# hrdkjain/GenIcoNet

Measured on AMD Instinct MI355X. Metric: meshes/sec training throughput, ico2ico I5 batch=36, higher is better.
Workload: dtype f32; 1 GPU; ico2ico AE training, I5, batch 36 per GPU (BASELINE configs[1]); per_gpu_batch=36, global_batch=36, subdivisions=5, parallelism=dp1

## Files before the change

geniconet_amd/_lib.py:

```python
import ctypes
import os

import numpy as np

_HERE = os.path.dirname(os.path.abspath(__file__))
LIB_PATH = os.environ.get('ICN_LIB_PATH') or os.path.join(_HERE, 'libicn.so')

OP_CONV_FWD, OP_CONV_BWD_DATA, OP_CONV_BWD_WEIGHT = 0, 1, 2
CORNER_MODES = {'zeros': 0, 'average': 1}
ABI_VERSION = 9
LAP_MODES = {'mean-v': 0, 'v-mean': 1, 'sum-kv': 2, 'kv-sum': 3}

_c_float_p = ctypes.c_void_p
_i32p = ctypes.POINTER(ctypes.c_int32)
_f32p = ctypes.POINTER(ctypes.c_float)
_intp = ctypes.POINTER(ctypes.c_int)

SIGNATURES = {
    'icn_abi_version': (ctypes.c_int, []),
    'icn_last_error': (ctypes.c_char_p, []),
    'icn_prepare_conv': (ctypes.c_int, [ctypes.c_int] * 3),
    'icn_prepare_upsample': (ctypes.c_int, [ctypes.c_int] * 2),
    'icn_conv_workspace_bytes': (ctypes.c_size_t, [ctypes.c_int] * 6),
    'icn_conv_fwd': (ctypes.c_int, [_c_float_p] * 4 + [ctypes.c_int] * 6 + [ctypes.c_void_p, ctypes.c_size_t, ctypes.c_void_p]),
# ... 23 lines not shown
    'icn_head_bwd': (ctypes.c_int, [_c_float_p] * 8 + [ctypes.c_int] * 3 + [ctypes.c_void_p]),
    'icn_p2p_loss_workspace_floats': (ctypes.c_size_t, [ctypes.c_int] * 2),
    'icn_p2p_loss_fwd': (ctypes.c_int, [_c_float_p] * 2 + [ctypes.c_int] * 2 + [ctypes.c_float] * 3 + [ctypes.c_int] + [_c_float_p] * 2 + [ctypes.c_void_p]),
    'icn_p2p_loss_bwd_workspace_floats': (ctypes.c_size_t, [ctypes.c_int] * 2),
    'icn_p2p_loss_bwd': (ctypes.c_int, [_c_float_p] * 3 + [ctypes.c_int] * 2 + [ctypes.c_float] * 3 + [ctypes.c_int] + [_c_float_p] * 2 + [ctypes.c_void_p]),
    'icn_mesh_reg_workspace_floats': (ctypes.c_size_t, [ctypes.c_int] * 2),
    'icn_mesh_reg_fwd': (ctypes.c_int, [_c_float_p] + [ctypes.c_int] * 2 + [ctypes.c_float] * 4 + [_c_float_p] * 2 + [ctypes.c_void_p]),
    'icn_mesh_reg_bwd_workspace_floats': (ctypes.c_size_t, [ctypes.c_int] * 2),
    'icn_mesh_reg_bwd': (ctypes.c_int, [_c_float_p] * 2 + [ctypes.c_int] * 2 + [ctypes.c_float] * 4 + [_c_float_p] * 2 + [ctypes.c_void_p]),
    'icn_kld_workspace_floats': (ctypes.c_size_t, [ctypes.c_size_t]),
    'icn_kld_fwd': (ctypes.c_int, [_c_float_p] * 2 + [ctypes.c_size_t] + [_c_float_p] * 2 + [ctypes.c_void_p]),
    'icn_kld_bwd': (ctypes.c_int, [_c_float_p] * 3 + [ctypes.c_size_t] + [_c_float_p] * 2 + [ctypes.c_void_p]),
    'icn_reparam_fwd': (ctypes.c_int, [_c_float_p] * 3 + [ctypes.c_size_t] + [_c_float_p] + [ctypes.c_void_p]),
    'icn_reparam_bwd': (ctypes.c_int, [_c_float_p] * 3 + [ctypes.c_size_t] + [_c_float_p] * 2 + [ctypes.c_void_p]),
    'icn_adam_step': (ctypes.c_int, [ctypes.c_int] + [ctypes.c_void_p] * 7 + [ctypes.c_double] * 4 + [ctypes.c_void_p]),
    'icn_adam_step_dev': (ctypes.c_int, [ctypes.c_int] + [ctypes.c_void_p] * 6 + [ctypes.c_double] * 4 + [ctypes.c_void_p]),
    'icn_table_stream_k': (ctypes.c_long, [ctypes.c_int] * 4 + [_i32p, ctypes.c_size_t]),
    'icn_table_tile_lists': (ctypes.c_long, [ctypes.c_int] * 7 + [_i32p, ctypes.c_size_t]),
    'icn_set_debug_flags': (ctypes.c_int, [ctypes.c_int]),
    'icn_device_status': (ctypes.c_int, [ctypes.c_int]),
    'icn_get_arith': (ctypes.c_int, []),
    'icn_set_arith': (ctypes.c_int, [ctypes.c_int]),
    'icn_build_flags': (ctypes.c_uint, []),
    'icn_host_selfcheck': (ctypes.c_long, [ctypes.c_int] * 2),
    'icn_debug_trace': (ctypes.c_int, [ctypes.c_void_p, ctypes.c_size_t]),
    'icn_point_to_mesh': (ctypes.c_int, [_c_float_p] * 3 + [ctypes.c_int] * 4 + [_c_float_p] * 3 + [ctypes.c_void_p]),
    'icn_point_to_mesh_bwd_workspace_bytes': (ctypes.c_size_t, [ctypes.c_int] * 4),
    'icn_point_to_mesh_grid_workspace_bytes': (ctypes.c_size_t, [ctypes.c_int] * 4),
    'icn_point_to_mesh_grid': (ctypes.c_int, [_c_float_p] * 3 + [ctypes.c_int] * 4 + [_c_float_p] * 3 + [ctypes.c_void_p, ctypes.c_size_t, ctypes.c_void_p]),
    'icn_point_to_mesh_bwd': (ctypes.c_int, [_c_float_p] * 6 + [ctypes.c_int] * 4 + [_c_float_p] * 2 + [ctypes.c_void_p, ctypes.c_size_t, ctypes.c_void_p]),
    'icn_table_conv_fwd': (ctypes.c_long, [ctypes.c_int] * 3 + [_i32p, ctypes.c_size_t]),
    'icn_table_wgrad7': (ctypes.c_long, [ctypes.c_int] * 3 + [_i32p, ctypes.c_size_t, ctypes.POINTER(ctypes.c_uint16), ctypes.c_size_t, _intp]),
    'icn_table_conv_bwd': (ctypes.c_long, [ctypes.c_int] * 3 + [_i32p, ctypes.c_size_t, _intp]),
    'icn_table_upsample': (ctypes.c_long, [ctypes.c_int] * 3 + [_i32p, _f32p, ctypes.c_size_t, _intp]),
    'icn_table_upsample_pairs': (ctypes.c_long, [ctypes.c_int, _i32p, ctypes.c_size_t]),
    'icn_table_faces': (ctypes.c_long, [ctypes.c_int, _i32p, ctypes.c_size_t]),
    'icn_table_vertex_stencils': (ctypes.c_long, [ctypes.c_int, _i32p, ctypes.c_size_t]),
    'icn_table_upconv_bwd': (ctypes.c_long, [ctypes.c_int] * 2 + [_i32p, _f32p, ctypes.c_size_t, _intp]),
    'icn_table_upconv': (ctypes.c_long, [ctypes.c_int, ctypes.c_int, _i32p, ctypes.c_size_t, _f32p, ctypes.c_size_t, _intp]),
}



class ProfileEntry(ctypes.Structure):
    _fields_ = [('kernel', ctypes.c_char_p), ('launches', ctypes.c_long), ('total_ms', ctypes.c_double),
                ('total_flops', ctypes.c_double)]


SIGNATURES['icn_profile_start'] = (ctypes.c_int, [ctypes.c_int])
SIGNATURES['icn_profile_stop'] = (ctypes.c_int, [ctypes.POINTER(ProfileEntry), ctypes.c_int])
SIGNATURES['icn_profile_select'] = (ctypes.c_int, [ctypes.c_char_p])

_lib = None


def lib():
    global _lib
    if _lib is None:
        if not os.path.exists(LIB_PATH):
            raise RuntimeError(
                'geniconet_amd: %s is missing -- the HIP extension is the product and has no fallback. '
                'Build it with `python -c "import __graft_entry__ as g; g.build()"` '
                '(or `make -C geniconet_amd/csrc`).' % LIB_PATH)
        handle = ctypes.CDLL(LIB_PATH)
        for name, (res, args) in SIGNATURES.items():
            fn = getattr(handle, name)
# ... 88 lines not shown
    n = L.icn_table_conv_fwd(r_in, stride, m, None, 0)
    if n < 0:
        check(-1, 'icn_table_conv_fwd')
    out = np.empty(n, dtype=np.int32)
    L.icn_table_conv_fwd(r_in, stride, m, out.ctypes.data_as(_i32p), n)
    return out.reshape(7, -1)


def table_wgrad7(r_in, stride, corner_mode):
    L, m = lib(), corner_code(corner_mode)
    meta = (ctypes.c_int * 2)()
    n = L.icn_table_wgrad7(r_in, stride, m, None, 0, None, 0, meta)
    if n < 0:
        check(-1, 'icn_table_wgrad7')
    if n == 0:
        return None
    U, npatch = meta[0], meta[1]
    rows, pos = np.empty(n, dtype=np.int32), np.empty(npatch * 16 * 8, dtype=np.uint16)
    L.icn_table_wgrad7(r_in, stride, m, rows.ctypes.data_as(_i32p), n, pos.ctypes.data_as(ctypes.POINTER(ctypes.c_uint16)), pos.size, meta)
    return rows.reshape(npatch, U), pos.reshape(npatch, 16, 8)


def table_conv_bwd(r_in, stride, corner_mode):
    L, m = lib(), corner_code(corner_mode)
    w = ctypes.c_int(0)
    n = L.icn_table_conv_bwd(r_in, stride, m, None, 0, ctypes.byref(w))
    if n < 0:
        check(-1, 'icn_table_conv_bwd')
    out = np.empty(n, dtype=np.int32)
    L.icn_table_conv_bwd(r_in, stride, m, out.ctypes.data_as(_i32p), n, ctypes.byref(w))
    return out.reshape(7, w.value, -1)


def table_upsample(r_in, corner_mode, transpose=False):
    L, m = lib(), corner_code(corner_mode)
    w = ctypes.c_int(0)
    n = L.icn_table_upsample(r_in, m, int(transpose), None, None, 0, ctypes.byref(w))
    if n < 0:
        check(-1, 'icn_table_upsample')
    idx, coef = np.empty(n, dtype=np.int32), np.empty(n, dtype=np.float32)
    L.icn_table_upsample(r_in, m, int(transpose), idx.ctypes.data_as(_i32p), coef.ctypes.data_as(_f32p), n, ctypes.byref(w))
    return idx.reshape(-1, w.value), coef.reshape(-1, w.value)


def table_faces(r):
    L = lib()
    n = L.icn_table_faces(r, None, 0)
    if n < 0:
        check(-1, 'icn_table_faces')
    out = np.empty(n, dtype=np.int32)
    L.icn_table_faces(r, out.ctypes.data_as(_i32p), n)
    return out.reshape(-1, 3)


def table_vertex_stencils(r):
    L = lib()
    n = L.icn_table_vertex_stencils(r, None, 0)
    if n < 0:
        check(-1, 'icn_table_vertex_stencils')
    out = np.empty(n, dtype=np.int32)
    L.icn_table_vertex_stencils(r, out.ctypes.data_as(_i32p), n)
    return out.reshape(-1, 6, 3)


def table_upsample_pairs(r_in):
    L = lib()
# ... 70 lines not shown
```

geniconet_amd/csrc/icn_api.cpp:

```cpp
#include <hip/hip_runtime.h>

#include <algorithm>
#include <cmath>
#include <cstdio>
#include <cstdlib>
#include <cstring>
#include <map>
#include <mutex>
#include <stdexcept>
#include <string>
#include <tuple>
#include <vector>

#include "../../include/icn.h"
#include "icn_geometry.h"
#include "icn_launch.h"
#include "icn_streamk.h"

namespace {

thread_local std::string g_err;

int fail(const std::string& msg) {
    g_err = msg;
// ... 17 lines not shown
        g_dry_elems += v.size();
        return d;
    }
    ICN_HIP(hipMalloc(reinterpret_cast<void**>(&d), v.size() * sizeof(T)));
    ICN_HIP(hipMemcpy(d, v.data(), v.size() * sizeof(T), hipMemcpyHostToDevice));
    return d;
}

struct DevDma {
    int32_t* code = nullptr;
    int32_t* slots = nullptr;
    int n_slots = 0, E = 1;
};
DevDma upload_dma(const std::vector<int32_t>& idx, int E, int P) {
    icn::DmaTable h;
    icn::build_dma_table(idx, E, P, h);
    DevDma d;
    d.code = upload(h.code);
    d.slots = upload(h.slots);
    d.n_slots = h.n_slots;
    d.E = E;
    return d;
}
struct ConvTables {
    int Pin = 0, Pout = 0, n_in = 0, n_out = 0, E = 1;
    int32_t* fwd = nullptr;
    int32_t* bwd = nullptr;
    int32_t* bwd1 = nullptr;
    int nv = 0, nvp = 0;
    int32_t* vidx = nullptr;
    int32_t* vorder = nullptr;
    uint32_t* vmask32 = nullptr;
    int32_t* vq = nullptr;
    int32_t* perm = nullptr;
    int32_t* bwd_perm = nullptr;
    uint32_t* mask32 = nullptr;
    std::vector<uint32_t> mask32_h;
    int key = 0;
    DevDma d_fwd, d_bwd, d_bwd1, d_virt, d_bwdp;
    int32_t* w7_rows = nullptr;
    uint16_t* w7_pos = nullptr;
    int w7_U = 0;
};
struct UpTables {
    int Pc = 0, Pf = 0, Wf = 0, Wb = 0;
    int32_t *idx_f = nullptr, *idx_b = nullptr;
    float *coef_f = nullptr, *coef_b = nullptr;
};

struct UpconvDev {
    int Pc = 0, Pf = 0, n_slots = 0, E = 1, nseg = 0;
    int seg_cnt[icn::UPCONV_MAX_SEG] = {}, seg_off[icn::UPCONV_MAX_SEG] = {};
    uint32_t seg_mask[icn::UPCONV_MAX_SEG] = {};
    int32_t *pix = nullptr, *code = nullptr, *slot_idx = nullptr;
    float *alpha = nullptr, *slot_coef = nullptr;
};

struct EllSplitDev {
    int W = 0, n_ovf = 0, W_ovf = 0;
    int32_t *idx = nullptr, *ovf_rows = nullptr, *ovf_idx = nullptr;
    float *coef = nullptr, *ovf_coef = nullptr;
};
EllSplitDev upload_ell_split(const icn::Ell& e, int W_main) {
    EllSplitDev d;
    const int W = e.width;
    d.W = W_main;
// ... 109 lines not shown
    std::vector<int32_t> fwd, bwd, perm;
    std::vector<uint8_t> mask;
    icn::build_conv_fwd(r_in, stride, mode, fwd);
    t.E = icn::build_conv_bwd(r_in, stride, mode, bwd);
    t.fwd = upload(fwd);
    t.bwd = upload(bwd);
    t.d_fwd = upload_dma(fwd, 1, t.Pout);
    t.d_bwd = upload_dma(bwd, t.E, t.Pin);
    {
        icn::DmaTable h;
        icn::build_dma_table(fwd, 1, t.Pout, h);
        icn::Wg7Table w7;
        if (icn::build_wgrad7(h, t.Pout, wgrad7_union_rows(stride), w7)) {
            t.w7_rows = upload(w7.urow);
            t.w7_pos = upload(w7.upos);
            t.w7_U = w7.U;
        }
    }
    std::vector<int32_t> primary;
    icn::VirtualRows vr;
    icn::split_conv_bwd(r_in, stride, bwd, t.E, primary, vr);
    t.bwd1 = upload(primary);
    t.d_bwd1 = upload_dma(primary, 1, t.Pin);
    t.nv = vr.nv;
    if (vr.nv > 0) {
        std::vector<int32_t> order, vidx_o;
        std::vector<uint8_t> vmask;
        icn::build_virtual_order(vr, t.nvp, order, vidx_o, vmask);
        t.vidx = upload(vidx_o);
        t.vorder = upload(order);
        t.vmask32 = upload(std::vector<uint32_t>(vmask.begin(), vmask.end()));
        t.d_virt = upload_dma(vidx_o, 1, t.nvp);
        t.vq = upload(vr.vq);
    }
    if (stride == 2) {
        icn::build_bwd_row_order(r_in, stride, bwd, t.E, perm, mask);
        t.perm = upload(perm);
        t.mask32_h.assign(mask.begin(), mask.end());
        t.mask32 = upload(t.mask32_h);
        t.key = 1 + ((r_in << 8) | (stride << 4) | mode);
        std::vector<int32_t> bwd_p(bwd.size());
        for (int te = 0; te < icn::NTAPS * t.E; ++te)
            for (int k = 0; k < t.Pin; ++k) bwd_p[(size_t)te * t.Pin + k] = bwd[(size_t)te * t.Pin + perm[k]];
        t.bwd_perm = upload(bwd_p);
        t.d_bwdp = upload_dma(bwd_p, t.E, t.Pin);
    }
    return t;
}
const ConvTables& conv_tables(int r_in, int stride, int mode) {
    int dev = 0;
    ICN_HIP(hipGetDevice(&dev));
    std::lock_guard<std::mutex> lk(g_mu);
    auto key = std::make_tuple(dev, r_in, stride, mode);
    auto it = g_conv.find(key);
    if (it != g_conv.end()) return it->second;
    return g_conv.emplace(key, make_conv_tables(r_in, stride, mode)).first->second;
}

std::map<std::pair<int, int>, int32_t*> g_vf;

const int32_t* vertex_faces(int r) {
    int dev = 0;
    ICN_HIP(hipGetDevice(&dev));
    std::lock_guard<std::mutex> lk(g_mu);
    auto key = std::make_pair(dev, r);
    auto it = g_vf.find(key);
// ... 298 lines not shown
    float* sk_part = reinterpret_cast<float*>(reinterpret_cast<char*>(sk_flag) + align256((size_t)icn::CONV_SK_FLAGS * sizeof(int)));
    icn::PrologueArgs p{};
    p.zero = sk_flag; p.n_zero = icn::CONV_SK_FLAGS;
    p.w = w0; p.w2 = w1; p.packed = wf; p.Cout = C0; p.Cout2 = C1; p.Cin = Cin; p.transpose = 0;
    p.bias = b0; p.bias2 = b1; p.bias_cat = bias_cat;
    p.src = x; p.slots = t.d_fwd.slots; p.side = side; p.n_slots = t.d_fwd.n_slots; p.E = 1; p.B = B; p.Ps = t.Pin; p.K = Cin;
    p.ns = t.n_in;
    icn::GatherGemmArgs a{};
    a.src = x; a.bias = w1 ? bias_cat : b0; a.dst = y0; a.dst2 = w1 ? y1 : nullptr; a.N0 = C0;
    a.idx = t.fwd; a.dcode = t.d_fwd.code; a.side = side; a.n_slots = t.d_fwd.n_slots;
    a.M = B * t.Pout; a.Ps = t.Pin; a.Pd = t.Pout; a.K = Cin; a.N = C; a.E = 1; a.ns = t.n_in;
    a.algo_flops = 2.0 * 7 * Cin * C * (double)B * t.Pout;
    a.sk_part = sk_part; a.sk_flag = sk_flag;
    choose_arith(a, p, wf, (size_t)7 * Cin * C, false);
    icn::launch_conv_prologue(p, s);
    icn::launch_gather_gemm_auto(a, s);
}

void conv_bwd_data_impl(const float* dy0, const float* dy1, const float* w0, const float* w1, float* dx, int B, int Cin, int C0,
                        int C1, int r_in, int stride, const ConvTables& t, void* ws, hipStream_t s) {
    const int C = C0 + C1;
    const size_t wbytes = wpack_bytes((size_t)7 * Cin * C);
    const TableCounts tc = table_counts(r_in, stride);
    const size_t side_bytes = align256((size_t)B * tc.slots_bwd * C0 * sizeof(float));
    float* wb = static_cast<float*>(ws);
    float* vout = reinterpret_cast<float*>(at(ws, wbytes));
    float* side = reinterpret_cast<float*>(at(ws, wbytes + align256((size_t)B * tc.nv * Cin * sizeof(float))));
    float* side2 = dy1 ? reinterpret_cast<float*>(reinterpret_cast<char*>(side) + side_bytes) : nullptr;
    int* sk_flag = reinterpret_cast<int*>(reinterpret_cast<char*>(side) + (dy1 ? 2 : 1) * side_bytes);
    float* sk_part = reinterpret_cast<float*>(reinterpret_cast<char*>(sk_flag) + align256((size_t)icn::CONV_SK_FLAGS * sizeof(int)));
    const bool split = stride == 1 && t.nv > 0 && t.nv * 8 < t.Pin;
    const DevDma& dm = split ? t.d_bwd1 : (stride == 2 ? t.d_bwdp : t.d_bwd);
    const DevDma& ds = split ? t.d_virt : dm;
    icn::PrologueArgs p{};
    p.w = w0; p.w2 = w1; p.packed = wb; p.Cout = C0; p.Cout2 = C1; p.Cin = Cin; p.transpose = 1;
    p.src = dy0; p.src2 = dy1; p.slots = ds.slots; p.side = side; p.side2 = side2; p.n_slots = ds.n_slots; p.E = ds.E; p.B = B;
    p.Ps = t.Pout; p.K = C0; p.ns = t.n_out;
    p.zero = sk_flag; p.n_zero = icn::CONV_SK_FLAGS;
    icn::GatherGemmArgs a{};
    a.src = dy0; a.src2 = dy1; a.dst = dx; a.N0 = Cin;
    a.idx = split ? t.bwd1 : (stride == 2 ? t.bwd_perm : t.bwd); a.dcode = dm.code; a.side = side; a.side2 = side2;
    a.n_slots = dm.n_slots; a.perm = t.perm; a.mask32 = t.mask32;
    a.mask32_host = t.mask32_h.empty() ? nullptr : t.mask32_h.data(); a.mask_key = t.key;
    a.M = B * t.Pin; a.Ps = t.Pout; a.Pd = t.Pin; a.K = C; a.N = Cin; a.E = split ? 1 : t.E; a.ns = t.n_out;
    a.algo_flops = 2.0 * 7 * Cin * C * (double)B * t.Pout;
    a.sk_part = sk_part; a.sk_flag = sk_flag;
    choose_arith(a, p, wb, (size_t)7 * Cin * C, split);
    icn::launch_conv_prologue(p, s);
    icn::launch_gather_gemm_auto(a, s);
    if (split) {
        icn::GatherGemmArgs v = a;
        v.wt = wb; v.arith_bn = 0;
        v.sk_part = nullptr; v.sk_flag = nullptr;
        v.dst = vout; v.idx = t.vidx; v.dcode = t.d_virt.code; v.n_slots = t.d_virt.n_slots; v.perm = t.vorder; v.mask32 = t.vmask32;
        v.M = B * t.nvp; v.Pd = t.nvp; v.E = 1;
        v.algo_flops = 0.0;
        icn::launch_gather_gemm_auto(v, s);
        icn::launch_row_scatter_add(vout, dx, t.vq, B, t.nv, t.nvp, t.Pin, Cin, s);
    }
}

void conv_bwd_weight_impl(const float* x, const float* dy0, const float* dy1, float* dw0, float* db0, float* dw1, float* db1, int B,
                          int Cin, int C0, int C1, const ConvTables& t, void* ws, hipStream_t s) {
    const int C = C0 + C1, M = B * t.Pout;
    float* partial = static_cast<float*>(ws);
    float* bpart = (db0 || db1) ? reinterpret_cast<float*>(at(ws, wgrad_partial_bytes(M, Cin, C, C0))) : nullptr;
    float* side = reinterpret_cast<float*>(at(ws, wgrad_partial_bytes(M, Cin, C, C0) + wgrad_bias_partial_bytes(M, Cin, C, C0)));
    const bool mfma = icn::wgrad_supported(Cin, C);
    if (mfma) {
        icn::PrologueArgs p{};
        p.Cin = Cin; p.src = x; p.slots = t.d_fwd.slots; p.side = side; p.n_slots = t.d_fwd.n_slots; p.E = 1; p.B = B; p.Ps = t.Pin;
        p.K = Cin; p.ns = t.n_in;
        icn::launch_conv_prologue(p, s);
    }
    icn::WgradArgs a{};
    a.x = x; a.dy = dy0; a.dy2 = dy1; a.Cout0 = C0; a.idx = t.fwd; a.dcode = mfma ? t.d_fwd.code : nullptr; a.side = side;
    a.n_slots = t.d_fwd.n_slots; a.partial = partial; a.bias_partial = bpart; a.dw = dw0; a.dbias = db0; a.dw2 = dw1; a.dbias2 = db1;
    a.M = M; a.Ps = t.Pin; a.Pd = t.Pout; a.Cin = Cin; a.Cout = C; a.ns = t.n_in;
    a.algo_flops = 2.0 * 7 * Cin * C * (double)M;
    a.w7_rows = t.w7_rows; a.w7_pos = t.w7_pos; a.w7_U = t.w7_U;
    icn::launch_wgrad(a, s);
}

}

namespace icn {
const char* const PROF_NAMES[PROF_KINDS] = {"k_conv_dma<128, 128, false>", "k_conv_dma<128, 64, false>", "k_conv_dma<64, 128, false>",
                                            "k_conv_dma<64, 64, false>",
                                            "k_gather_gemm<128, 128>", "k_gather_gemm<128, 64>", "k_gather_gemm<64, 128>",
                                            "k_gather_gemm<64, 64>", "k_wgrad_dma<128, 128>", "k_wgrad_dma<128, 64>",
                                            "k_wgrad_dma<64, 128>", "k_wgrad_dma<64, 64>", "k_wgrad<128, 128>", "k_wgrad<128, 64>",
                                            "k_wgrad<64, 128>", "k_wgrad<64, 64>", "k_conv_dma<128, 128, true>",
                                            "k_conv_dma<128, 64, true>", "k_conv_dma<64, 128, true>", "k_conv_dma<64, 64, true>",
                                            "k_conv_dma_sk<64, 128, false>", "k_conv_dma_sk<64, 64, false>", "k_conv_dma_sk<64, 128, true>",
                                            "k_conv_dma_sk<64, 64, true>", "k_wgrad7",
                                            "k_conv_dma8<64, 128, false>", "k_conv_dma8<64, 128, true>", "k_conv_dma_sk8<64, 128, false>",
                                            "k_conv_dma_sk8<64, 128, true>", "k_conv_dense_sk<64, 128>", "k_conv_dense_sk<64, 64>", "k_conv_single_sk<64, 128>",
                                            "k_conv_single_sk<64, 64>", "k_wgrad_dense<128, 128>", "k_wgrad_dense<128, 64>",
                                            "k_wgrad_dense<64, 128>", "k_wgrad_dense<64, 64>",
                                            "k_conv_b3_sk<128, 128, 8>", "k_conv_b3_sk<128, 64, 4>", "k_conv_b3_dense_sk<128, 128, 8>",
                                            "k_conv_b3_dense_sk<128, 64, 4>", "k_wgrad7<.., 1>", "k_wgrad_dma<.., 1>", "k_wgrad_dense<.., 1>", "k_conv_b3<128, BN, NW>",
                                            "k_conv_b3_single_sk<128, 128, 8>", "k_conv_b3_single_sk<128, 64, 4>",
                                            "k_point_to_mesh", "k_point_to_mesh_bwd_point", "k_point_to_mesh_bwd_vertex",
                                            "k_p2m_grid_bounds", "k_p2m_grid_count", "k_p2m_grid_scan", "k_p2m_grid_fill",
                                            "k_p2m_grid_query"};
void prof_mark_begin(int kind, double flops, hipStream_t s) {
    if (!g_prof_on) return;
    g_prof_mu.lock();
    if (!g_prof_on || g_prof_used >= g_prof.size() || (g_prof_only >= 0 && kind != g_prof_only)) { g_prof_mu.unlock(); return; }
    ProfRec& r = g_prof[g_prof_used];
    r.kind = kind;
    r.flops = flops;
    (void)hipEventRecord(r.e0, s);
    g_prof_open = true;
}
void prof_mark_end(hipStream_t s) {
    if (!g_prof_open) return;
    (void)hipEventRecord(g_prof[g_prof_used].e1, s);
    ++g_prof_used;
    g_prof_open = false;
    g_prof_mu.unlock();
}
}

extern "C" {

int icn_profile_start(int max_launches) {
    try {
        if (max_launches < 1) throw std::invalid_argument("icn_profile_start: max_launches must be positive");
        std::lock_guard<std::mutex> lk(g_prof_mu);
        while ((int)g_prof.size() < max_launches) {
            ProfRec r{};
            ICN_HIP(hipEventCreate(&r.e0));
            ICN_HIP(hipEventCreate(&r.e1));
            g_prof.push_back(r);
        }
        g_prof_used = 0;
        g_prof_on = true;
// ... 893 lines not shown

long icn_table_conv_fwd(int r_in, int stride, int corner_mode, int32_t* out, size_t cap) {
    try {
        std::vector<int32_t> v;
        icn::build_conv_fwd(r_in, stride, corner_mode, v);
        if (out) std::memcpy(out, v.data(), std::min(cap, v.size()) * sizeof(int32_t));
        return (long)v.size();
    } catch (const std::exception& e) {
        return fail(e.what());
    }
}

long icn_table_wgrad7(int r_in, int stride, int corner_mode, int32_t* rows, size_t cap_rows, uint16_t* pos, size_t cap_pos, int* meta) {
    try {
        std::vector<int32_t> fwd;
        icn::build_conv_fwd(r_in, stride, corner_mode, fwd);
        const int P = (int)(fwd.size() / icn::NTAPS);
        icn::DmaTable h;
        icn::build_dma_table(fwd, 1, P, h);
        icn::Wg7Table w7;
        if (!icn::build_wgrad7(h, P, wgrad7_union_rows(stride), w7)) {
            if (meta) meta[0] = meta[1] = 0;
            return 0;
        }
        if (meta) { meta[0] = w7.U; meta[1] = w7.npatch; }
        if (rows) std::memcpy(rows, w7.urow.data(), std::min(cap_rows, w7.urow.size()) * sizeof(int32_t));
        if (pos) std::memcpy(pos, w7.upos.data(), std::min(cap_pos, w7.upos.size()) * sizeof(uint16_t));
        return (long)w7.urow.size();
    } catch (const std::exception& e) {
        return fail(e.what());
    }
}

long icn_table_conv_bwd(int r_in, int stride, int corner_mode, int32_t* out, size_t cap, int* width) {
    try {
        std::vector<int32_t> v;
        const int E = icn::build_conv_bwd(r_in, stride, corner_mode, v);
        if (width) *width = E;
        if (out) std::memcpy(out, v.data(), std::min(cap, v.size()) * sizeof(int32_t));
        return (long)v.size();
    } catch (const std::exception& e) {
        return fail(e.what());
    }
}

long icn_table_upsample(int r_in, int corner_mode, int transpose, int32_t* idx, float* coef, size_t cap, int* width) {
    try {
        icn::Ell f, b;
        icn::build_upsample(r_in, corner_mode, f, b);
        const icn::Ell& e = transpose ? b : f;
        if (width) *width = e.width;
        if (idx) std::memcpy(idx, e.idx.data(), std::min(cap, e.idx.size()) * sizeof(int32_t));
        if (coef) std::memcpy(coef, e.coef.data(), std::min(cap, e.coef.size()) * sizeof(float));
        return (long)e.idx.size();
    } catch (const std::exception& e) {
        return fail(e.what());
    }
}

long icn_table_upsample_pairs(int r_in, int32_t* out, size_t cap) {
    try {
        std::vector<int32_t> v;
        icn::build_upsample_pairs(r_in, v);
        if (out) std::memcpy(out, v.data(), std::min(cap, v.size()) * sizeof(int32_t));
        return (long)v.size();
    } catch (const std::exception& e) {
// ... 68 lines not shown
```

geniconet_amd/csrc/icn_geometry.cpp:

```cpp
#include "icn_geometry.h"

#include <algorithm>
#include <cstdlib>
#include <array>
#include <cmath>
#include <map>
#include <stdexcept>

namespace icn {

const int TAP_DA[NTAPS] = {0, 1, 0, -1, -1, 0, 1};
const int TAP_DB[NTAPS] = {0, 0, 1, 1, 0, -1, -1};

namespace {

struct Pt {
    int c, a, b;
};

inline Pt prev1(int, Pt p) { return {(p.c + 4) % 5, p.a + p.b, -p.a}; }
inline Pt prev2(int n, Pt p) { return {(p.c + 4) % 5, p.a + n, p.b - n}; }
inline Pt prev3(int n, Pt p) { return {(p.c + 4) % 5, 3 * n - p.b, p.a + p.b - n}; }
inline Pt next1(int, Pt p) { return {(p.c + 1) % 5, -p.b, p.a + p.b}; }
inline Pt next2(int n, Pt p) { return {(p.c + 1) % 5, p.a - n, p.b + n}; }
// ... 120 lines not shown
        }
        for (size_t l = 0; l < levels; ++l) {
            std::array<int32_t, NTAPS> row;
            for (int t = 0; t < NTAPS; ++t) row[t] = l < leftover[t].size() ? leftover[t][l] : IDX_ZERO;
            rows.push_back(row);
            vr.vq.push_back(q);
        }
    }
    vr.nv = (int)rows.size();
    vr.vidx.assign((size_t)NTAPS * std::max(vr.nv, 1), IDX_ZERO);
    for (int v = 0; v < vr.nv; ++v)
        for (int t = 0; t < NTAPS; ++t) vr.vidx[(size_t)t * vr.nv + v] = rows[v][t];
}

void build_virtual_order(const VirtualRows& vr, int& nvp, std::vector<int32_t>& order, std::vector<int32_t>& vidx_o,
                         std::vector<uint8_t>& mask32) {
    const int nv = vr.nv;
    nvp = (nv + 31) / 32 * 32;
    std::vector<unsigned> taps(nv, 0);
    for (int v = 0; v < nv; ++v)
        for (int t = 0; t < NTAPS; ++t)
            if (vr.vidx[(size_t)t * nv + v] != IDX_ZERO) taps[v] |= 1u << t;
    order.resize(nvp);
    for (int k = 0; k < nvp; ++k) order[k] = k;
    std::stable_sort(order.begin(), order.begin() + nv, [&](int x, int y) { return taps[x] < taps[y]; });
    vidx_o.assign((size_t)NTAPS * nvp, IDX_ZERO);
    mask32.assign(nvp / 32, 0);
    for (int k = 0; k < nv; ++k) {
        for (int t = 0; t < NTAPS; ++t) vidx_o[(size_t)t * nvp + k] = vr.vidx[(size_t)t * nv + order[k]];
        mask32[k / 32] |= (uint8_t)taps[order[k]];
    }
}

void build_dma_table(const std::vector<int32_t>& idx, int E, int P, DmaTable& out) {
    out.E = E;
    out.n_slots = 0;
    out.code.assign((size_t)NTAPS * P, IDX_ZERO);
    out.slots.clear();
    std::map<std::vector<int32_t>, int> slot_of;
    std::vector<int32_t> ent;
    for (int t = 0; t < NTAPS; ++t)
        for (int p = 0; p < P; ++p) {
            ent.clear();
            for (int e = 0; e < E; ++e) {
                const int32_t c = idx[((size_t)t * E + e) * P + p];
                if (c != IDX_ZERO) ent.push_back(c);
            }
            int32_t code = IDX_ZERO;
            if (ent.size() == 1 && ent[0] >= 0) {
                code = ent[0];
            } else if (!ent.empty()) {
                ent.resize(E, IDX_ZERO);
                auto it = slot_of.find(ent);
                if (it == slot_of.end()) {
                    it = slot_of.emplace(ent, out.n_slots++).first;
                    out.slots.insert(out.slots.end(), ent.begin(), ent.end());
                }
                code = -2 - it->second;
            }
            out.code[(size_t)t * P + p] = code;
        }
}

bool build_wgrad7(const DmaTable& d, int P, int max_U, Wg7Table& out) {
    out = Wg7Table{};
    if (P <= 0 || P % WG7_PX != 0 || (size_t)NTAPS * P != d.code.size()) return false;
// ... 401 lines not shown
```

geniconet_amd/csrc/icn_geometry.h:

```cpp
#pragma once
#include <cstdint>
#include <vector>

namespace icn {

enum CornerMode { CORNER_ZEROS = 0, CORNER_AVERAGE = 1 };

constexpr int32_t IDX_ZERO = -1;
constexpr int32_t IDX_POLE = -2;

constexpr int NTAPS = 7;
extern const int TAP_DA[NTAPS];
extern const int TAP_DB[NTAPS];

inline int pixels(int r) { return 10 << (2 * r); }

void build_conv_fwd(int r_in, int stride, int corner_mode, std::vector<int32_t>& out);

int build_conv_bwd(int r_in, int stride, int corner_mode, std::vector<int32_t>& out);

struct VirtualRows {
    int nv = 0;
    std::vector<int32_t> vidx;
    std::vector<int32_t> vq;
};
void split_conv_bwd(int r_in, int stride, const std::vector<int32_t>& bwd_idx, int E, std::vector<int32_t>& primary,
                    VirtualRows& vr);

void build_virtual_order(const VirtualRows& vr, int& nvp, std::vector<int32_t>& order, std::vector<int32_t>& vidx_o,
                         std::vector<uint8_t>& mask32);

struct DmaTable {
    int n_slots = 0, E = 1;
    std::vector<int32_t> code;
    std::vector<int32_t> slots;
};
void build_dma_table(const std::vector<int32_t>& idx, int E, int P, DmaTable& out);

constexpr int WG7_PX = 16;
constexpr int WG7_ROW_BYTES = 256;
struct Wg7Table {
    int U = 0, npatch = 0;
    std::vector<int32_t> urow;
    std::vector<uint16_t> upos;
};
bool build_wgrad7(const DmaTable& d, int P, int max_U, Wg7Table& out);

struct Ell {
    int rows = 0, width = 0;
    std::vector<int32_t> idx;
    std::vector<float> coef;
};
void build_upsample(int r_in, int corner_mode, Ell& fwd, Ell& bwd);
void build_upsample_pairs(int r_in, std::vector<int32_t>& out);

constexpr int UPCONV_REGULAR = 19;
constexpr int UPCONV_TAPS = UPCONV_REGULAR + NTAPS;
constexpr int UPCONV_MAX_SEG = 5;
struct UpconvTable {
    int Pc = 0, Pf = 0;
    std::vector<float> alpha;
    int nseg = 0;
    int seg_cnt[UPCONV_MAX_SEG] = {};
// ... 24 lines not shown
```

geniconet_amd/csrc/icn_kernels.hip:

```cpp
#include <hip/hip_runtime.h>
#include <stdint.h>

#include <algorithm>
#include <cfloat>
#include <atomic>
#include <cstdio>
#include <cstdlib>
#include <cstring>
#include <map>
#include <mutex>
#include <tuple>
#include <vector>
#include <stdexcept>
#include <type_traits>
#include <utility>

#include "icn_launch.h"
#include "icn_streamk.h"

#ifndef ICN_CHAIN_PRIO
#define ICN_CHAIN_PRIO 0
#endif
#if ICN_CHAIN_PRIO > 0
#define ICN_CHAIN_SETPRIO() __builtin_amdgcn_s_setprio(ICN_CHAIN_PRIO)
// ... 3059 lines not shown
}

void launch_conv_generic(const float* src, const float* w, const float* bias, float* dst, const int32_t* idx, int B, int Ps,
                         int Pd, int K, int N, int E, int ns, int transpose, hipStream_t s) {
    const size_t total = (size_t)B * Pd * N;
    const int blocks = (int)std::min((size_t)16384, (total + 255) / 256);
    hipLaunchKernelGGL(k_conv_generic, dim3(blocks), dim3(256), 0, s, src, w, bias, dst, idx, B, Ps, Pd, K, N, E, ns,
                       transpose);
}

__global__ void k_row_scatter_add(const float* __restrict__ src, float* __restrict__ dst, const int32_t* __restrict__ q, int B,
                                  int nv, int nvp, int P, int C) {
    const int c4n = C / 4;
    const size_t total = (size_t)B * nv * c4n;
    for (size_t i = (size_t)blockIdx.x * blockDim.x + threadIdx.x; i < total; i += (size_t)gridDim.x * blockDim.x) {
        const int c = (int)(i % c4n) * 4;
        const size_t bv = i / c4n;
        const int v = (int)(bv % nv), b = (int)(bv / nv);
        const int32_t qv = q[v];
        if (v > 0 && q[v - 1] == qv) continue;
        float* d = dst + ((size_t)b * P + qv) * C + c;
        f32x4 acc = ld4(d);
        for (int k = v; k < nv && q[k] == qv; ++k) acc += ld4(src + ((size_t)b * nvp + k) * C + c);
        *reinterpret_cast<f32x4*>(d) = acc;
    }
}

void launch_row_scatter_add(const float* src, float* dst, const int32_t* q, int B, int nv, int nvp, int P, int C, hipStream_t s) {
    const size_t total = (size_t)B * nv * (C / 4);
    hipLaunchKernelGGL(k_row_scatter_add, dim3((unsigned)std::min((size_t)4096, (total + 255) / 256)), dim3(256), 0, s, src, dst, q, B,
                       nv, nvp, P, C);
}

__global__ __launch_bounds__(256) void k_upconv_prologue(UpconvPrologueArgs a, int npack) {
    if ((int)blockIdx.x < npack) {
        const int Ct = a.Cout + a.Cout2, total = a.NV * Ct * a.Cin;
        for (int i = blockIdx.x * 256 + threadIdx.x; i < total; i += npack * 256) {
            const int ci = i % a.Cin, co = (i / a.Cin) % Ct, v = i / (a.Cin * Ct);
            const float* wp = co < a.Cout ? a.w + ((size_t)co * a.Cin + ci) * 7 : a.w2 + ((size_t)(co - a.Cout) * a.Cin + ci) * 7;
            float acc = 0.f;
#pragma unroll
            for (int t = 0; t < 7; ++t) acc += a.alpha[v * 7 + t] * wp[t];
            a.packed[i] = acc;
        }
        if (a.bias_cat && blockIdx.x == 0)
            for (int c = threadIdx.x; c < Ct; c += 256) a.bias_cat[c] = c < a.Cout ? a.bias[c] : a.bias2[c - a.Cout];
        return;
    }
    const int j = blockIdx.x - npack;
    const int b = j / a.n_slots, sl = j % a.n_slots;
    for (int ch = 4 * threadIdx.x; ch < a.Cin; ch += 4 * 256) {
        f32x4 v = {0.f, 0.f, 0.f, 0.f};
        for (int e = 0; e < a.E; ++e) {
            const int32_t c = a.slot_idx[sl * a.E + e];
            if (c >= 0) v += a.slot_coef[sl * a.E + e] * ld4(a.src + ((size_t)b * a.Ps + c) * a.Cin + ch);
        }
        *reinterpret_cast<f32x4*>(a.side + ((size_t)b * a.n_slots + sl) * a.Cin + ch) = v;
    }
}

void launch_upconv_prologue(const UpconvPrologueArgs& a, hipStream_t s) {
    const int npack = std::min(4096, (a.NV * (a.Cout + a.Cout2) * a.Cin + 255) / 256);
    const int nside = (a.side && a.n_slots > 0) ? a.B * a.n_slots : 0;
    hipLaunchKernelGGL(k_upconv_prologue, dim3(npack + nside), dim3(256), 0, s, a, npack);
}

// ... 10 lines not shown
```

geniconet_amd/csrc/icn_launch.h:

```cpp
#pragma once
#include <hip/hip_runtime.h>
#include <stdint.h>

namespace icn {

constexpr int MAX_SEGS = 5;
struct RowSegs {
    int nseg;
    int B;
    int row0[MAX_SEGS], cnt[MAX_SEGS], off[MAX_SEGS];
    unsigned mask[MAX_SEGS];
};

struct GatherGemmArgs {
    const float* src;
    const float* src2;
    const float* wt;
    const float* bias;
    float* dst;
    float* dst2;
    int N0;
    const int32_t* idx;
    const int32_t* dcode;
    const float* side;
// ... 60 lines not shown
bool wgrad_pair_supported(int M, int Ps, int Pd, int Cin, int Cout0, int Cout1);
int wgrad_splits(int M, int Cin, int Cout, int Cout0 = 0);
int wgrad7_splits(int M, int Pd, int Cin, int Cout, int Cout0);
void launch_wgrad(const WgradArgs& a, hipStream_t s);
bool stem_supported(int Cin, int Cout);
void launch_stem_fwd(const float* x, const float* w, const float* bias, float* y, const int32_t* idx, int M, int Ps, int Pd,
                     int Cin, int Cout, int ns, hipStream_t s);

void launch_upconv_gather(const float* dy0, const float* dy1, float* g, const int32_t* idx, const float* coef, const int32_t* rows,
                          int B, int Pin, int nrows, int rows_total, int C0, int C1, int W, int acc, hipStream_t s);

struct PatchTab { const int32_t* prow; const uint16_t* plocal; int npatch, umax, gridW; };
bool upconv_patch_usable(const PatchTab& t, int B, size_t rows_per_sample, int C0, int C1);
void launch_upconv_scatter_lds(const float* z, const float* bias, float* y0, float* y1, const PatchTab& t, const float* coef, int B,
                               int zrows, int Pout, int C0, int C1, hipStream_t s);
void launch_upconv_gather_lds(const float* dy0, const float* dy1, float* g, const PatchTab& t, const int32_t* cls,
                              const float* cls_coef, int ncls, int B, int Pin, int Pc, int C0, int C1, hipStream_t s);

constexpr int UPCONV_PX_CLASSES = 32;
void launch_upconv_gather_px(const float* dy0, const float* dy1, float* g, const int32_t* srcs, const int32_t* cls,
                             const float* cls_coef, int ncls, int B, int Pin, int Pc, int C0, int C1, hipStream_t s);

void launch_upconv_scatter(const float* z, const float* bias, float* y0, float* y1, const int32_t* idx, const float* coef,
                           const int32_t* rows, int B, int zrows, int nrows, int Pout, int C0, int C1, int W, int acc, hipStream_t s);

void launch_spmm_ell(const float* in, float* out, const int32_t* idx, const float* coef, int B, int Pin, int Pout, int C,
                     int W, hipStream_t s);

void launch_conv_generic(const float* src, const float* w, const float* bias, float* dst, const int32_t* idx, int B, int Ps,
                         int Pd, int K, int N, int E, int ns, int transpose, hipStream_t s);

void launch_row_scatter_add(const float* src, float* dst, const int32_t* q, int B, int nv, int nvp, int P, int C, hipStream_t s);

struct PrologueArgs {
    const float* w; const float* w2; float* packed; int Cout, Cout2, Cin, transpose;
    const float* bias; const float* bias2; float* bias_cat;
    const float* src; const float* src2; const int32_t* slots; float* side; float* side2; int n_slots, E, B, Ps, K, ns;
    int* zero; int n_zero;
    int b3_flat_n;
    void* packed_b3; int b3_bn;
};
void launch_conv_prologue(const PrologueArgs& a, hipStream_t s);

struct UpconvPrologueArgs {
    const float* w; const float* w2; float* packed; int Cout, Cout2, Cin, NV; const float* alpha;
    const float* bias; const float* bias2; float* bias_cat;
    const float* src; const int32_t* slot_idx; const float* slot_coef; float* side; int n_slots, E, B, Ps;
};
void launch_upconv_prologue(const UpconvPrologueArgs& a, hipStream_t s);

bool bn_supported(int C);
int bn_chunks(int M);
void launch_bn_stats(const float* x, int M, int C, float eps, float momentum, float* running_mean, float* running_var, float* stat,
                     float* ws, hipStream_t s);
void launch_bn_stats2(const float* a, const float* b, int M, int C, float eps_a, float mom_a, float* rm_a, float* rv_a, float* stat_a,
                      float eps_b, float mom_b, float* rm_b, float* rv_b, float* stat_b, float* ws, hipStream_t s);
void launch_bn_relu_fwd(const float* a, const float* b, const float* stat_a, const float* stat_b, const float* ga, const float* ba,
                        const float* gb, const float* bb, float* y, int M, int C, hipStream_t s);
void launch_bn_relu_bwd(const float* dy, const float* a, const float* b, const float* stat_a, const float* stat_b, const float* ga,
                        const float* ba, const float* gb, const float* bb, float* da, float* db, float* sums, float* ws, int M, int C,
                        float* dbeta_a, float* dgamma_a, float* dbeta_b, float* dgamma_b, hipStream_t s);

bool head_supported(int Cin, int Cout);
int head_chunks(int M);
void launch_head_fwd(const float* x, const float* w, const float* bias, float* y, int M, int Cin, int Cout, hipStream_t s);
void launch_head_bwd(const float* dy, const float* y, const float* x, const float* w, float* dx, float* dw, float* db, float* ws,
// ... 15 lines not shown
void launch_kld_fwd(const float* mu, const float* logvar, size_t n, float* out, float* partial, hipStream_t s);
void launch_kld_bwd(const float* mu, const float* logvar, const float* upstream, size_t n, float* dmu, float* dlogvar, hipStream_t s);
void launch_reparam_fwd(const float* mu, const float* logvar, const float* eps, size_t n, float* z, hipStream_t s);
void launch_reparam_bwd(const float* dz, const float* logvar, const float* eps, size_t n, float* dmu, float* dlogvar, hipStream_t s);

void launch_point_to_mesh(const float* pts, const float* vts, const int32_t* faces, int B, int P, int V, int F, float* dist,
                          int32_t* face, int32_t* kind, hipStream_t s);
size_t point_to_mesh_bwd_record_bytes(int B, int P);
void launch_point_to_mesh_bwd(const float* pts, const float* vts, const int32_t* faces, const int32_t* face, const int32_t* kind,
                              const float* ddist, int B, int P, int V, int F, float* dpts, float* dvts, void* ws, hipStream_t s);

int p2m_grid_res(int F);
size_t point_to_mesh_grid_bytes(int B, int F);
hipError_t launch_point_to_mesh_grid(const float* pts, const float* vts, const int32_t* faces, int B, int P, int V, int F, float* dist,
                                     int32_t* face, int32_t* kind, void* ws, hipStream_t s);

int debug_flags();
int set_debug_flags(int flags);

enum ProfKind { PROF_DMA_128x128 = 0, PROF_DMA_128x64, PROF_DMA_64x128, PROF_DMA_64x64, PROF_GG_128x128, PROF_GG_128x64,
                PROF_GG_64x128, PROF_GG_64x64, PROF_WGD_128x128, PROF_WGD_128x64, PROF_WGD_64x128, PROF_WGD_64x64, PROF_WG_128x128,
                PROF_WG_128x64, PROF_WG_64x128, PROF_WG_64x64,
                PROF_DMAS_128x128, PROF_DMAS_128x64, PROF_DMAS_64x128, PROF_DMAS_64x64,
                PROF_DMAK_64x128, PROF_DMAK_64x64, PROF_DMAKS_64x128, PROF_DMAKS_64x64,
                PROF_WG7,
                PROF_DMA8_64x128, PROF_DMAS8_64x128, PROF_DMAK8_64x128, PROF_DMAKS8_64x128,
                PROF_DENSEK_64x128, PROF_DENSEK_64x64,
                PROF_SINGLEK_64x128, PROF_SINGLEK_64x64,
                PROF_WGDENSE_128x128, PROF_WGDENSE_128x64, PROF_WGDENSE_64x128, PROF_WGDENSE_64x64,
                PROF_B3K_128x128, PROF_B3K_128x64, PROF_B3DENSEK_128x128, PROF_B3DENSEK_128x64,
                PROF_WG7_B3, PROF_WGD_B3, PROF_WGDENSE_B3, PROF_B3_MASKED, PROF_B3SINGLEK_128x128, PROF_B3SINGLEK_128x64,
                PROF_P2M, PROF_P2M_BWD_POINT, PROF_P2M_BWD_VERTEX,
                PROF_P2M_GRID_BOUNDS, PROF_P2M_GRID_COUNT, PROF_P2M_GRID_SCAN, PROF_P2M_GRID_FILL, PROF_P2M_GRID_QUERY,
                PROF_KINDS };
extern const char* const PROF_NAMES[PROF_KINDS];
void prof_mark_begin(int kind, double flops, hipStream_t s);
void prof_mark_end(hipStream_t s);

constexpr int ADAM_MAX_TENSORS = 96;
void launch_adam(int count, float* const* p, const float* const* g, float* const* m, float* const* v, const size_t* numel,
                 const float* step_size, const float* bc2_sqrt, double beta1, double beta2, double eps, double weight_decay, hipStream_t s,
                 const float* scal_dev = nullptr);

}
```

include/icn.h:

```cpp
#ifndef ICN_H
#define ICN_H

#include <stddef.h>
#include <stdint.h>

#ifdef __cplusplus
extern "C" {
#endif

#define ICN_ABI_VERSION 9

#define ICN_CORNER_ZEROS 0
#define ICN_CORNER_AVERAGE 1

#define ICN_IDX_ZERO (-1)
#define ICN_IDX_POLE (-2)

#define ICN_OP_CONV_FWD 0
#define ICN_OP_CONV_BWD_DATA 1
#define ICN_OP_CONV_BWD_WEIGHT 2

int icn_abi_version(void);
const char* icn_last_error(void);

// ... 72 lines not shown
size_t icn_mesh_reg_bwd_workspace_floats(int B, int r);
int icn_mesh_reg_bwd(const float* grid, const float* upstream, int B, int r, float f_edge, float f_ncons, float f_smooth,
                     float edge_length, float* dgrid, float* ws, void* stream);

size_t icn_kld_workspace_floats(size_t n);
int icn_kld_fwd(const float* mu, const float* logvar, size_t n, float* out, float* ws, void* stream);
int icn_kld_bwd(const float* mu, const float* logvar, const float* upstream, size_t n, float* dmu, float* dlogvar, void* stream);

int icn_reparam_fwd(const float* mu, const float* logvar, const float* eps, size_t n, float* z, void* stream);
int icn_reparam_bwd(const float* dz, const float* logvar, const float* eps, size_t n, float* dmu, float* dlogvar, void* stream);

int icn_point_to_mesh(const float* points, const float* vertices, const int32_t* faces, int B, int P, int V, int F, float* dist2,
                      int32_t* face, int32_t* kind, void* stream);

size_t icn_point_to_mesh_bwd_workspace_bytes(int B, int P, int V, int F);
int icn_point_to_mesh_bwd(const float* points, const float* vertices, const int32_t* faces, const int32_t* face, const int32_t* kind,
                          const float* ddist, int B, int P, int V, int F, float* dpoints, float* dvertices, void* ws, size_t ws_bytes,
                          void* stream);

size_t icn_point_to_mesh_grid_workspace_bytes(int B, int P, int V, int F);
int icn_point_to_mesh_grid(const float* points, const float* vertices, const int32_t* faces, int B, int P, int V, int F, float* dist2,
                           int32_t* face, int32_t* kind, void* ws, size_t ws_bytes, void* stream);

int icn_adam_step(int count, float* const* params, const float* const* grads, float* const* exp_avg, float* const* exp_avg_sq,
                  const size_t* numel, const float* step_size, const float* bc2_sqrt, double beta1, double beta2, double eps,
                  double weight_decay, void* stream);

int icn_adam_step_dev(int count, float* const* params, const float* const* grads, float* const* exp_avg, float* const* exp_avg_sq,
                      const size_t* numel, const float* scalars_dev, double beta1, double beta2, double eps, double weight_decay,
                      void* stream);

long icn_table_conv_fwd(int r_in, int stride, int corner_mode, int32_t* out, size_t cap);
long icn_table_conv_bwd(int r_in, int stride, int corner_mode, int32_t* out, size_t cap, int* width);
long icn_table_upsample(int r_in, int corner_mode, int transpose, int32_t* idx, float* coef, size_t cap, int* width);
long icn_table_upsample_pairs(int r_in, int32_t* out, size_t cap);
long icn_table_faces(int r, int32_t* out, size_t cap);
long icn_table_vertex_stencils(int r, int32_t* out, size_t cap);
long icn_table_stream_k(int ntiles, int grid, int nk, int ku, int32_t* out, size_t cap);
long icn_table_tile_lists(int r_in, int stride, int corner_mode, int B, int bm, int ntn, int grid, int32_t* out, size_t cap);
long icn_table_upconv(int r_in, int corner_mode, int32_t* ints, size_t cap_ints, float* floats, size_t cap_floats, int* meta);
long icn_table_upconv_bwd(int r_in, int corner_mode, int32_t* idx, float* coef, size_t cap, int* width);

long icn_table_wgrad7(int r_in, int stride, int corner_mode, int32_t* rows, size_t cap_rows, uint16_t* pos, size_t cap_pos, int* meta);

typedef struct icn_profile_entry {
    const char* kernel;
    long launches;
    double total_ms;
    double total_flops;
} icn_profile_entry;
int icn_profile_start(int max_launches);
int icn_profile_stop(icn_profile_entry* out, int cap);
int icn_profile_select(const char* kernel);

int icn_set_debug_flags(int flags);

int icn_debug_trace(void* device_buffer, size_t n_u64);

long icn_host_selfcheck(int r, int corner_mode);

#define ICN_STATUS_STREAMK_LOST 1
int icn_device_status(int clear);

#define ICN_ARITH_F32 0
#define ICN_ARITH_BF16X3 1
int icn_get_arith(void);
// ... 9 lines not shown
```

Before: 5629 meshes/s.

## Handle stride-1 conv backward virtual rows with a single owner-grouped kernel

```diff
diff --git a/geniconet_amd/_lib.py b/geniconet_amd/_lib.py
--- a/geniconet_amd/_lib.py
+++ b/geniconet_amd/_lib.py
@@ -79,6 +79,7 @@
     'icn_table_conv_fwd': (ctypes.c_long, [ctypes.c_int] * 3 + [_i32p, ctypes.c_size_t]),
     'icn_table_wgrad7': (ctypes.c_long, [ctypes.c_int] * 3 + [_i32p, ctypes.c_size_t, ctypes.POINTER(ctypes.c_uint16), ctypes.c_size_t, _intp]),
     'icn_table_conv_bwd': (ctypes.c_long, [ctypes.c_int] * 3 + [_i32p, ctypes.c_size_t, _intp]),
+    'icn_table_virtual_rows': (ctypes.c_long, [ctypes.c_int] * 2 + [_i32p, ctypes.c_size_t, _intp]),
     'icn_table_upsample': (ctypes.c_long, [ctypes.c_int] * 3 + [_i32p, _f32p, ctypes.c_size_t, _intp]),
     'icn_table_upsample_pairs': (ctypes.c_long, [ctypes.c_int, _i32p, ctypes.c_size_t]),
     'icn_table_faces': (ctypes.c_long, [ctypes.c_int, _i32p, ctypes.c_size_t]),
@@ -233,6 +234,23 @@
     return out.reshape(7, w.value, -1)
 
 
+def table_virtual_rows(r_in, corner_mode):
+    L, m = lib(), corner_code(corner_mode)
+    meta = (ctypes.c_int * 3)()
+    n = L.icn_table_virtual_rows(r_in, m, None, 0, meta)
+    if n < 0:
+        check(-1, 'icn_table_virtual_rows')
+    nv, n_own, n_ent = list(meta)
+    out = np.empty(n, dtype=np.int32)
+    L.icn_table_virtual_rows(r_in, m, out.ctypes.data_as(_i32p), n, meta)
+    o = [0, nv, 8 * nv if nv else nv, 0, 0, 0]
+    o[3] = o[2] + n_own
+    o[4] = o[3] + n_own + 1
+    o[5] = o[4] + 2 * n_ent
+    return dict(vq=out[:o[1]], vidx=out[o[1]:o[2]].reshape(7, -1), own_q=out[o[2]:o[3]], own_off=out[o[3]:o[4]],
+                ent=out[o[4]:o[5]].reshape(-1, 2))
+
+
 def table_upsample(r_in, corner_mode, transpose=False):
     L, m = lib(), corner_code(corner_mode)
     w = ctypes.c_int(0)
diff --git a/geniconet_amd/csrc/icn_api.cpp b/geniconet_amd/csrc/icn_api.cpp
--- a/geniconet_amd/csrc/icn_api.cpp
+++ b/geniconet_amd/csrc/icn_api.cpp
@@ -73,6 +73,8 @@
     int32_t* vorder = nullptr;
     uint32_t* vmask32 = nullptr;
     int32_t* vq = nullptr;
+    int n_own = 0;
+    int32_t *vown_q = nullptr, *vown_off = nullptr, *vent = nullptr;
     int32_t* perm = nullptr;
     int32_t* bwd_perm = nullptr;
     uint32_t* mask32 = nullptr;
@@ -248,6 +250,12 @@
         t.vmask32 = upload(std::vector<uint32_t>(vmask.begin(), vmask.end()));
         t.d_virt = upload_dma(vidx_o, 1, t.nvp);
         t.vq = upload(vr.vq);
+        icn::VirtualOwners vo;
+        icn::build_virtual_owners(vr, vo);
+        t.n_own = (int)vo.own_q.size();
+        t.vown_q = upload(vo.own_q);
+        t.vown_off = upload(vo.own_off);
+        t.vent = upload(vo.ent);
     }
     if (stride == 2) {
         icn::build_bwd_row_order(r_in, stride, bwd, t.E, perm, mask);
@@ -612,9 +620,11 @@
     const bool split = stride == 1 && t.nv > 0 && t.nv * 8 < t.Pin;
     const DevDma& dm = split ? t.d_bwd1 : (stride == 2 ? t.d_bwdp : t.d_bwd);
     const DevDma& ds = split ? t.d_virt : dm;
+    const bool one_launch = split && !(icn::debug_flags() & 524288) && icn::virt_rows_supported(C, C0, Cin);
     icn::PrologueArgs p{};
     p.w = w0; p.w2 = w1; p.packed = wb; p.Cout = C0; p.Cout2 = C1; p.Cin = Cin; p.transpose = 1;
     p.src = dy0; p.src2 = dy1; p.slots = ds.slots; p.side = side; p.side2 = side2; p.n_slots = ds.n_slots; p.E = ds.E; p.B = B;
+    if (one_launch) { p.slots = nullptr; p.side = nullptr; p.side2 = nullptr; p.n_slots = 0; }
     p.Ps = t.Pout; p.K = C0; p.ns = t.n_out;
     p.zero = sk_flag; p.n_zero = icn::CONV_SK_FLAGS;
     icn::GatherGemmArgs a{};
@@ -628,7 +638,12 @@
     choose_arith(a, p, wb, (size_t)7 * Cin * C, split);
     icn::launch_conv_prologue(p, s);
     icn::launch_gather_gemm_auto(a, s);
-    if (split) {
+    if (one_launch) {
+        icn::VirtRowsArgs v{};
+        v.dy0 = dy0; v.dy1 = dy1; v.wt = wb; v.dx = dx; v.own_q = t.vown_q; v.own_off = t.vown_off; v.ent = t.vent;
+        v.n_own = t.n_own; v.B = B; v.Ps = t.Pout; v.Pd = t.Pin; v.K = C; v.Ks = C0; v.N = Cin; v.ns = t.n_out;
+        icn::launch_virt_rows(v, s);
+    } else if (split) {
         icn::GatherGemmArgs v = a;
         v.wt = wb; v.arith_bn = 0;
         v.sk_part = nullptr; v.sk_flag = nullptr;
@@ -683,7 +698,7 @@
                                             "k_conv_b3_single_sk<128, 128, 8>", "k_conv_b3_single_sk<128, 64, 4>",
                                             "k_point_to_mesh", "k_point_to_mesh_bwd_point", "k_point_to_mesh_bwd_vertex",
                                             "k_p2m_grid_bounds", "k_p2m_grid_count", "k_p2m_grid_scan", "k_p2m_grid_fill",
-                                            "k_p2m_grid_query"};
+                                            "k_p2m_grid_query", "k_virt_rows"};
 void prof_mark_begin(int kind, double flops, hipStream_t s) {
     if (!g_prof_on) return;
     g_prof_mu.lock();
@@ -1643,6 +1658,27 @@
     }
 }
 
+long icn_table_virtual_rows(int r_in, int corner_mode, int32_t* out, size_t cap, int* meta) {
+    try {
+        std::vector<int32_t> bwd, primary, v;
+        const int E = icn::build_conv_bwd(r_in, 1, corner_mode, bwd);
+        icn::VirtualRows vr;
+        icn::split_conv_bwd(r_in, 1, bwd, E, primary, vr);
+        icn::VirtualOwners vo;
+        icn::build_virtual_owners(vr, vo);
+        if (meta) { meta[0] = vr.nv; meta[1] = (int)vo.own_q.size(); meta[2] = (int)(vo.ent.size() / 2); }
+        v.insert(v.end(), vr.vq.begin(), vr.vq.end());
+        if (vr.nv > 0) v.insert(v.end(), vr.vidx.begin(), vr.vidx.end());
+        v.insert(v.end(), vo.own_q.begin(), vo.own_q.end());
+        v.insert(v.end(), vo.own_off.begin(), vo.own_off.end());
+        v.insert(v.end(), vo.ent.begin(), vo.ent.end());
+        if (out) std::memcpy(out, v.data(), std::min(cap, v.size()) * sizeof(int32_t));
+        return (long)v.size();
+    } catch (const std::exception& e) {
+        return fail(e.what());
+    }
+}
+
 long icn_table_conv_bwd(int r_in, int stride, int corner_mode, int32_t* out, size_t cap, int* width) {
     try {
         std::vector<int32_t> v;
diff --git a/geniconet_amd/csrc/icn_geometry.cpp b/geniconet_amd/csrc/icn_geometry.cpp
--- a/geniconet_amd/csrc/icn_geometry.cpp
+++ b/geniconet_amd/csrc/icn_geometry.cpp
@@ -176,6 +176,24 @@
     }
 }
 
+void build_virtual_owners(const VirtualRows& vr, VirtualOwners& out) {
+    out = VirtualOwners{};
+    for (int v = 0; v < vr.nv; ++v) {
+        if (v > 0 && vr.vq[v] < vr.vq[v - 1]) throw std::logic_error("icn: virtual rows are not sorted by their pixel");
+        if (v == 0 || vr.vq[v] != vr.vq[v - 1]) {
+            out.own_q.push_back(vr.vq[v]);
+            out.own_off.push_back((int32_t)(out.ent.size() / 2));
+        }
+        for (int t = 0; t < NTAPS; ++t) {
+            const int32_t c = vr.vidx[(size_t)t * vr.nv + v];
+            if (c == IDX_ZERO) continue;
+            out.ent.push_back(t);
+            out.ent.push_back(c);
+        }
+    }
+    out.own_off.push_back((int32_t)(out.ent.size() / 2));
+}
+
 void build_dma_table(const std::vector<int32_t>& idx, int E, int P, DmaTable& out) {
     out.E = E;
     out.n_slots = 0;
diff --git a/geniconet_amd/csrc/icn_geometry.h b/geniconet_amd/csrc/icn_geometry.h
--- a/geniconet_amd/csrc/icn_geometry.h
+++ b/geniconet_amd/csrc/icn_geometry.h
@@ -29,6 +29,13 @@
 
 void build_virtual_order(const VirtualRows& vr, int& nvp, std::vector<int32_t>& order, std::vector<int32_t>& vidx_o,
                          std::vector<uint8_t>& mask32);
+
+struct VirtualOwners {
+    std::vector<int32_t> own_q;
+    std::vector<int32_t> own_off;
+    std::vector<int32_t> ent;
+};
+void build_virtual_owners(const VirtualRows& vr, VirtualOwners& out);
 
 struct DmaTable {
     int n_slots = 0, E = 1;
diff --git a/geniconet_amd/csrc/icn_kernels.hip b/geniconet_amd/csrc/icn_kernels.hip
--- a/geniconet_amd/csrc/icn_kernels.hip
+++ b/geniconet_amd/csrc/icn_kernels.hip
@@ -3115,6 +3115,74 @@
                        nv, nvp, P, C);
 }
 
+constexpr int VR_BS = 48;
+constexpr int VR_LD = 36;
+__global__ __launch_bounds__(256) void k_virt_rows(VirtRowsArgs a) {
+    __shared__ __attribute__((aligned(16))) float sW[64 * VR_LD];
+    __shared__ __attribute__((aligned(16))) float sY[VR_BS * VR_LD];
+    const int tid = threadIdx.x, cn = tid & 15, sg = tid >> 4;
+    const int o = blockIdx.x, n0 = blockIdx.y * 64, b0 = blockIdx.z * VR_BS;
+    const int nb = min(VR_BS, a.B - b0);
+    const int q = a.own_q[o], e0 = a.own_off[o], e1 = a.own_off[o + 1];
+    float acc[3][4] = {};
+    for (int e = e0; e < e1; ++e) {
+        const int t = a.ent[2 * e], code = a.ent[2 * e + 1];
+        for (int k0 = 0; k0 < a.K; k0 += 32) {
+            __syncthreads();
+#pragma unroll
+            for (int i = tid; i < 64 * 8; i += 256) {
+                const int row = i >> 3, c4 = i & 7;
+                *reinterpret_cast<f32x4*>(&sW[row * VR_LD + 4 * c4]) = ld4(a.wt + ((size_t)t * a.N + n0 + row) * a.K + k0 + 4 * c4);
+            }
+            const float* src = k0 < a.Ks ? a.dy0 : a.dy1;
+            const int kk = k0 < a.Ks ? k0 : k0 - a.Ks;
+            for (int i = tid; i < nb * 8; i += 256) {
+                const int sm = i >> 3, c4 = i & 7;
+                f32x4 v = {0.f, 0.f, 0.f, 0.f};
+                if (code >= 0) v = ld4(src + ((size_t)(b0 + sm) * a.Ps + code) * a.Ks + kk + 4 * c4);
+                else if (code <= -2) v = pole_mean4(src, b0 + sm, a.Ps, a.ns, -2 - code, a.Ks, kk + 4 * c4);
+                *reinterpret_cast<f32x4*>(&sY[sm * VR_LD + 4 * c4]) = v;
+            }
+            __syncthreads();
+#pragma unroll
+            for (int c4 = 0; c4 < 8; ++c4) {
+                f32x4 w[4];
+#pragma unroll
+                for (int j = 0; j < 4; ++j) w[j] = *reinterpret_cast<const f32x4*>(&sW[(cn + 16 * j) * VR_LD + 4 * c4]);
+#pragma unroll
+                for (int i = 0; i < 3; ++i) {
+                    if (sg + 16 * i >= nb) continue;
+                    const f32x4 y = *reinterpret_cast<const f32x4*>(&sY[(sg + 16 * i) * VR_LD + 4 * c4]);
+#pragma unroll
+                    for (int j = 0; j < 4; ++j) {
+                        acc[i][j] = fmaf(y[0], w[j][0], acc[i][j]);
+                        acc[i][j] = fmaf(y[1], w[j][1], acc[i][j]);
+                        acc[i][j] = fmaf(y[2], w[j][2], acc[i][j]);
+                        acc[i][j] = fmaf(y[3], w[j][3], acc[i][j]);
+                    }
+                }
+            }
+        }
+    }
+#pragma unroll
+    for (int i = 0; i < 3; ++i) {
+        if (sg + 16 * i >= nb) continue;
+        float* d = a.dx + ((size_t)(b0 + sg + 16 * i) * a.Pd + q) * a.N + n0 + cn;
+#pragma unroll
+        for (int j = 0; j < 4; ++j) d[16 * j] += acc[i][j];
+    }
+}
+
+bool virt_rows_supported(int K, int Ks, int N) { return N % 64 == 0 && K % 32 == 0 && Ks % 32 == 0 && Ks >= 32 && (K == Ks || K == 2 * Ks); }
+
+void launch_virt_rows(const VirtRowsArgs& a, hipStream_t s) {
+    if (a.n_own <= 0) return;
+    static_assert((64 + VR_BS) * VR_LD * 4 <= 24 * 1024, "k_virt_rows must fit beside two k_wgrad7 workgroups");
+    prof_mark_begin(PROF_VIRT_ROWS, 0.0, s);
+    hipLaunchKernelGGL(k_virt_rows, dim3((unsigned)a.n_own, (unsigned)(a.N / 64), (unsigned)((a.B + VR_BS - 1) / VR_BS)), dim3(256), 0, s, a);
+    prof_mark_end(s);
+}
+
 __global__ __launch_bounds__(256) void k_upconv_prologue(UpconvPrologueArgs a, int npack) {
     if ((int)blockIdx.x < npack) {
         const int Ct = a.Cout + a.Cout2, total = a.NV * Ct * a.Cin;
diff --git a/geniconet_amd/csrc/icn_launch.h b/geniconet_amd/csrc/icn_launch.h
--- a/geniconet_amd/csrc/icn_launch.h
+++ b/geniconet_amd/csrc/icn_launch.h
@@ -116,6 +116,16 @@
 
 void launch_row_scatter_add(const float* src, float* dst, const int32_t* q, int B, int nv, int nvp, int P, int C, hipStream_t s);
 
+struct VirtRowsArgs {
+    const float* dy0; const float* dy1;
+    const float* wt;
+    float* dx;
+    const int32_t* own_q; const int32_t* own_off; const int32_t* ent;
+    int n_own, B, Ps, Pd, K, Ks, N, ns;
+};
+bool virt_rows_supported(int K, int Ks, int N);
+void launch_virt_rows(const VirtRowsArgs& a, hipStream_t s);
+
 struct PrologueArgs {
     const float* w; const float* w2; float* packed; int Cout, Cout2, Cin, transpose;
     const float* bias; const float* bias2; float* bias_cat;
@@ -197,6 +207,7 @@
                 PROF_WG7_B3, PROF_WGD_B3, PROF_WGDENSE_B3, PROF_B3_MASKED, PROF_B3SINGLEK_128x128, PROF_B3SINGLEK_128x64,
                 PROF_P2M, PROF_P2M_BWD_POINT, PROF_P2M_BWD_VERTEX,
                 PROF_P2M_GRID_BOUNDS, PROF_P2M_GRID_COUNT, PROF_P2M_GRID_SCAN, PROF_P2M_GRID_FILL, PROF_P2M_GRID_QUERY,
+                PROF_VIRT_ROWS,
                 PROF_KINDS };
 extern const char* const PROF_NAMES[PROF_KINDS];
 void prof_mark_begin(int kind, double flops, hipStream_t s);
diff --git a/include/icn.h b/include/icn.h
--- a/include/icn.h
+++ b/include/icn.h
@@ -128,6 +128,7 @@
 
 long icn_table_conv_fwd(int r_in, int stride, int corner_mode, int32_t* out, size_t cap);
 long icn_table_conv_bwd(int r_in, int stride, int corner_mode, int32_t* out, size_t cap, int* width);
+long icn_table_virtual_rows(int r_in, int corner_mode, int32_t* out, size_t cap, int* meta);
 long icn_table_upsample(int r_in, int corner_mode, int transpose, int32_t* idx, float* coef, size_t cap, int* width);
 long icn_table_upsample_pairs(int r_in, int32_t* out, size_t cap);
 long icn_table_faces(int r, int32_t* out, size_t cap);
```

After: 5678 meshes/s, median of 6. No clear change (+0.9%).
